# jsourati/nn-active-learning

Measured on AMD Instinct MI355X. Metric: patches/sec Fisher-scored (32^3, 2-class), higher is better.
Workload: dtype f32 (fp32 operands split into 16-bit pieces on the 16-bit MFMA, fp32 accumulate: fp16 pairs - 22-23 bits kept per operand, three products - in the conv under the head (forward + backward), in dec1's forward launch and in the other backward launches; bf16 triples - all 24 bits, exact, six products -

## Files before the change

### nn-active-learning_amd/csrc/alq_internal.h

```cpp
#pragma once
#include <hip/hip_runtime.h>

#include <cstdint>
#include <cstdio>
#include <memory>
#include <string>
#include <vector>

#include "alq.h"

namespace alq {

void set_error(const char *fmt, ...);

#define ALQ_HIP(expr)                                                                     \
    do {                                                                                  \
        hipError_t e_ = (expr);                                                           \
        if (e_ != hipSuccess) {                                                           \
            ::alq::set_error("%s:%d: %s -> %s", __FILE__, __LINE__, #expr,               \
                             hipGetErrorString(e_));                                      \
            return ALQ_EHIP;                                                              \
        }                                                                                 \
    } while (0)

// ... 192 lines not shown
    int mask_split = 0;
    long long mask_delta = 0;
    const unsigned char *mask_bits = nullptr;
    unsigned char *sign_out = nullptr;
    const unsigned *in_bits = nullptr;
    const float *in_vec = nullptr;
    float in_vec_amax = 0.f;
    const unsigned *in_vec16 = nullptr;
    unsigned *out_amax = nullptr;
    int amax_from = 0;
    const unsigned *in_amax = nullptr, *in_amax2 = nullptr;
    float in_bound = 0.f;
    const float *fc_W = nullptr;
    long long fc_F = 0;
    float *fc_part = nullptr;
    unsigned *fc_bits = nullptr;
    unsigned *flip_cnt = nullptr, *flip_list = nullptr;
    int flip_cap = 0;
    float flip_l1 = 0.f;
    bool flip_bias_nonzero = false;
};

extern unsigned long long *g_igemm2_dbg;
constexpr int ALQ_NKNOBS = 10;
extern int g_dbg_knobs[ALQ_NKNOBS];
extern int g_dcp_last_form;
extern int g_no_f16x2;
extern int g_no_fixed;
extern int g_no_xcd_order;
int igemm2_build_plan(const IgemmPlan &p1, Igemm2Plan *p2);
void igemm2_pack_weights(Igemm2Plan *p2, const std::vector<float> &Bmat);
int igemm2_launch(alq_ctx *ctx, const Igemm2Plan &plan, const View &in, const View &out, const float *bias,
                  int relu, int accumulate, int N, int prof_cls, const Igemm2Fuse *fuse);

struct Igemm3Plan {
    bool ok = false;
    bool wres = false;
    int NTW = 1;
    int wgs_per_cu = 1;
    size_t lds_bytes = 0;
    std::vector<unsigned short> h_W;
    void *d_W = nullptr;
    std::vector<unsigned short> h_W16;
    void *d_W16 = nullptr;
    int w16_exp = 0;
};
int igemm3_build_plan(const Igemm2Plan &p2, Igemm3Plan *p3);
// ... 111 lines not shown
                   const float *fc_W, float *fc_part, float *asum_part, unsigned char *fc_bits, float flip_tau);
int c3d_bwd_build(const View &fwd_in, const View &fwd_out, const int k[3], const int lo[3], const int s[3], C3dPlan *plan);
void c3d_bwd_pack(C3dPlan *plan, const std::vector<float> &Bmat_fwd );
void c3d_presplit_vec(const float *v, long long F, int e, std::vector<unsigned short> *out);
int c3d_bwd_launch(alq_ctx *ctx, const C3dPlan &plan, int N, const unsigned char *bits, const void *vec16, int e_in, const unsigned char *maskA,
                   float *dB, float *sumA, float *sumB, int rows_per_wave = 8);

struct T3dPlan {
    bool ok = false;
    int kind = 0;
    int w_exp = 0;
    double flops_per_patch = 0;
    std::vector<unsigned short> h_W;
    void *d_W = nullptr;
};
int t3d_build(const View &in, const View &out, const int k[3], const int lo[3], const int s[3], T3dPlan *fwd, T3dPlan *bwd);
void t3d_fwd_pack(T3dPlan *plan, const float *W );
void t3d_bwd_pack(T3dPlan *plan, const float *W);
void t3d8_fwd_pack(T3dPlan *plan, const float *W );
void t3d8_bwd_pack(T3dPlan *plan, const float *W );
int t3d8_bwd_launch(alq_ctx *ctx, const T3dPlan &plan, const View &dout, const View &din, int N, float in_bound, const unsigned char *mask_bits, float *dsum);
int t3d_fwd_launch(alq_ctx *ctx, const T3dPlan &plan, const View &in, const View &out, const float *bias, int N, float *osum, unsigned *out_amax);
int t3d_bwd_launch(alq_ctx *ctx, const T3dPlan &plan, const View &dout, const View &din, int N, float in_bound, const unsigned char *mask_bits,
                   float *dsum);

struct E3dPlan {
    bool ok = false;
    int w_exp = 0;
    double flops_per_patch = 0;
    std::vector<unsigned short> h_Whi, h_Wlo;
    void *d_Whi = nullptr, *d_Wlo = nullptr;
};
int e3d_build(const View &in, const View &out, const int k[3], const int lo[3], const int s[3], E3dPlan *plan);
void e3d_pack(E3dPlan *plan, const float *W );
int e3d_bwd_launch(alq_ctx *ctx, const E3dPlan &plan, int N, const float *skip, const float *dpool, const unsigned char *am2, const unsigned char *sg2,
                   const unsigned char *am1, const unsigned char *sg1, float *dsum2, float *dsum1, float in_bound,
                   bool rows );

struct D3dPlan {
    bool ok = false;
    int w_exp = 0;
    double flops_per_patch = 0;
    std::vector<unsigned short> h_Whi, h_Wlo;
    void *d_Whi = nullptr, *d_Wlo = nullptr;
    std::vector<unsigned short> h_Bhi, h_Blo;
    void *d_Bhi = nullptr, *d_Blo = nullptr;
};
// ... 222 lines not shown
```

### nn-active-learning_amd/csrc/igemm2.hip

```cpp
#include "alq_internal.h"

#include <algorithm>
#include <cmath>
#include <cstring>

namespace alq {

typedef float f32x4 __attribute__((ext_vector_type(4)));
typedef float f32x2 __attribute__((ext_vector_type(2)));

#ifdef ALQ_STAMPS
#define STAMP(var) asm volatile("s_memtime %0\n\ts_waitcnt lgkmcnt(0)" : "=s"(var)::"memory")
#define PHASE_END(idx)                         \
    do {                                       \
        unsigned long long t_now_;             \
        STAMP(t_now_);                         \
        ph[idx] += t_now_ - t_last;            \
        t_last = t_now_;                       \
    } while (0)
#else
#define PHASE_END(idx) do {} while (0)
#endif

constexpr int I2_CBP = 12;
// ... 461 lines not shown
}

void igemm2_pack_weights(Igemm2Plan *p2, const std::vector<float> &Bmat) {
    const Igemm2Args &a = p2->a;
    const int NTW = p2->NTW, Ci = a.Ci, Co = a.Co;
    p2->h_W.assign((size_t)a.nchunks * a.ntaps * NTW * 128, 0.f);
    for (int ch = 0; ch < a.nchunks; ++ch)
        for (int tp = 0; tp < a.ntaps; ++tp)
            for (int nt = 0; nt < NTW; ++nt)
                for (int lane = 0; lane < 64; ++lane)
                    for (int s = 0; s < 2; ++s) {
                        const int c = ch * 8 + 2 * (lane >> 4) + s;
                        const int co = nt * 16 + (lane & 15);
                        if (co < Co)
                            p2->h_W[((((size_t)ch * a.ntaps + tp) * NTW + nt) * 64 + lane) * 2 + s] =
                                Bmat[((size_t)tp * Ci + c) * Co + co];
                    }
}

unsigned long long *g_igemm2_dbg = nullptr;
int g_no_f16x2 = 0;
int g_no_xcd_order = 0;
int g_no_fixed = 0;
int g_dbg_knobs[ALQ_NKNOBS] = {0, 0, 0, 0, 0, 0, 0, 0, 0, 0};

template <int NTW, bool WRES, int GEO, bool SUMS>
static int launch2_s(alq_ctx *ctx, const Igemm2Plan &plan, const Igemm2Args &a, unsigned grid) {
    auto kfn = igemm2_kernel<NTW, WRES, GEO, SUMS>;
    if (plan.lds_bytes > 64 * 1024)
        ALQ_HIP(hipFuncSetAttribute(reinterpret_cast<const void *>(kfn), hipFuncAttributeMaxDynamicSharedMemorySize,
                                    (int)plan.lds_bytes));
    hipLaunchKernelGGL(kfn, dim3(grid), dim3(256), plan.lds_bytes, ctx->stream, a);
    ALQ_HIP(hipGetLastError());
    return ALQ_OK;
}

template <int NTW, bool WRES, int GEO>
static int launch2_t(alq_ctx *ctx, const Igemm2Plan &plan, const Igemm2Args &a, unsigned grid) {
    return (a.osumA || a.osumB) ? launch2_s<NTW, WRES, GEO, true>(ctx, plan, a, grid)
                                : launch2_s<NTW, WRES, GEO, false>(ctx, plan, a, grid);
}

int igemm2_launch(alq_ctx *ctx, const Igemm2Plan &plan, const View &in, const View &out, const float *bias, int relu,
                  int accumulate, int N, int prof_cls, const Igemm2Fuse *fuse) {
    Igemm2Args a = plan.a;
    ALQ_REQUIRE(in.C == a.Ci && in.D == a.ID && in.H == a.IH && in.W == a.IW, ALQ_EINVAL,
                "igemm2: input view does not match plan");
// ... 53 lines not shown
```

### nn-active-learning_amd/csrc/model.hip

```cpp
#include <algorithm>
#include <cmath>
#include <cstdarg>
#include <cstring>
#include <string>
#include <memory>

#include "alq_internal.h"

namespace alq {

static thread_local char g_err[1024] = "";
void set_error(const char *fmt, ...) {
    va_list ap;
    va_start(ap, fmt);
    vsnprintf(g_err, sizeof(g_err), fmt, ap);
    va_end(ap);
}

int gather_normalize_impl(alq_ctx *, const void *const *, int, int, const int64_t[3], const int64_t[3],
                          const int64_t *, int64_t, const int32_t[3], const double *, int, int, void *);
int score_entropy_impl(alq_ctx *, const float *, int64_t, double *, float *);
int synth_impl(alq_ctx *, uint64_t, int64_t, int64_t, int64_t, float *);
int gather_rows_impl(alq_ctx *, const float *, const int64_t *, int64_t, int64_t, float *);
int debug_view_copy(alq_ctx *, const View &, int, float *);
// ... 91 lines not shown
    int no_flipfix = 0;
    size_t amax_tiles_len = 0;
    int in_dims[4] = {1, 1, 1, 1};
    int nclass = 0;
    int L = 0;
    std::vector<Layer> layers;
    std::vector<void *> allocs;
    float *logits = nullptr, *dlogits = nullptr, *post = nullptr;
    double *S = nullptr, *sizes = nullptr, *Apart = nullptr;
    double *Spart = nullptr;
    int *nslab = nullptr;
    int nslab_max = 1;
    float *wg_partial = nullptr;
    size_t wg_partial_len = 0;
    double *gn_partial = nullptr;
    size_t gn_partial_len = 0;
    double *df_scratch = nullptr;
    double *ls_part = nullptr;
    std::vector<int> ls_nslab;
    int ls_nslab_max = 0;
    int last_lsum = 0;
    float *x_stage = nullptr;
    int64_t epp = 0;
    int knobs[ALQ_NKNOBS] = {0, 0, 0, 0, 0, 0, 0, 0, 0, 0};
    int no_f16x2 = 0;
    int no_xcd_order = 0;
    int requested_batch = 0;
    int no_bound16 = 0;
    int no_fixed = 0;
    int no_presplit = 0;
    int no_signs = 0;
    int no_signs0 = 0;
    int f16_fwd_mask = -1;
    int f16_fwd_derived = 0;
    int no_f16_derived = 0;
    float *d_bound_L = nullptr, *d_bound_B = nullptr;
    int *d_bound_src = nullptr;
    int no_light_kernels = 0;
    int no_c3d = 0;
    int c3_bwd_rows = 8;
    bool last_c3 = false;
    bool last_c3_bwd = false;
    int no_e3d = 0;
    int last_e3b = 0;
    int e3d_rows = 0;
    int last_e3b_form = 0;
    int no_d3d = 0;
    int last_d3f = 0;
    int no_f3d = 0, last_f3f = 0;
    int no_d3b = 0, last_d3b = 0;
    int no_t3d = 0;
    int last_dcp = 0;
    int last_t3f = 0, last_t3b = 0;
    bool last_f16_derived = false;
    int64_t host_pack_elems = 0;
    void *d_wscal = nullptr;
    bool hv_ready = false;
    double *hv_part = nullptr;
    double *hv_p64 = nullptr;

    template <typename T>
    int dalloc(T **p, size_t count) {
        void *q = nullptr;
        const size_t bytes = std::max<size_t>(count * sizeof(T), 256);
        if (hipMalloc(&q, bytes) != hipSuccess) {
            set_error("hipMalloc of %zu bytes failed", bytes);
            return ALQ_ENOMEM;
        }
        allocs.push_back(q);
// ... 35 lines not shown
            s.pool.push_back(pr.first);
            s.pool.push_back(pr.second);
        }
        s.pending.clear();
    }
    return ALQ_OK;
}

static int upload1(alq_model *m, IgemmPlan *p) {
    if (!p->d_W) ALQ_TRY(m->dalloc(&p->d_W, p->h_W.size()));
    ALQ_HIP(hipMemcpyAsync(p->d_W, p->h_W.data(), p->h_W.size() * sizeof(float), hipMemcpyHostToDevice,
                           m->ctx->stream));
    if (p->smallc) {
        if (!p->d_koff) ALQ_TRY(m->dalloc(&p->d_koff, p->h_koff.size()));
        ALQ_HIP(hipMemcpyAsync(p->d_koff, p->h_koff.data(), p->h_koff.size() * sizeof(int),
                               hipMemcpyHostToDevice, m->ctx->stream));
    }
    ALQ_HIP(hipStreamSynchronize(m->ctx->stream));
    std::vector<float>().swap(p->h_W);
    return ALQ_OK;
}

static bool g_use_v2 = true;
static int g_knob_override[ALQ_NKNOBS] = {-1, -1, -1, -1, -1, -1, -1, -1, -1, -1};

static void apply_knobs(const alq_model *m) {
    for (int k = 0; k < ALQ_NKNOBS; ++k) g_dbg_knobs[k] = g_knob_override[k] >= 0 ? g_knob_override[k] : m->knobs[k];
    g_no_f16x2 = m->no_f16x2;
    g_no_xcd_order = m->no_xcd_order;
    g_no_fixed = m->no_fixed;
}

static int gemm_build(const ConvDesc &d, int max_batch, Gemm *g, const G4Geom *g4 = nullptr) {
    ALQ_TRY(igemm_build_plan(d, max_batch, &g->p1));
    if (g4 && !getenv("ALQ_DISABLE_V4")) {
        G4Geom gg = *g4;
        gg.flops_per_patch = g->p1.flops_per_patch;
        ALQ_TRY(igemm4_build_plan(gg, max_batch, &g->p4));
    }
    ALQ_TRY(igemm2_build_plan(g->p1, &g->p2));
    ALQ_TRY(direct_build_plan(g->p1, &g->pd));
    if (!g_use_v2) { g->p2.ok = false; g->pd.ok = false; }
    ALQ_TRY(igemm3_build_plan(g->p2, &g->p3));
    if (d.ID == 1 && d.IH == 1 && d.IW == 1 && d.tz.size() == 1 && d.sm == 1 && d.so == 1 && !getenv("ALQ_NO_FCGEMM"))
        ALQ_TRY(fcgemm_build_plan(d.Ci, d.Co, &g->pfc));
    if (const char *e = getenv("ALQ_DISABLE_V3")) { if (e[0] == '1') g->p3.ok = false; }
    return ALQ_OK;
// ... 911 lines not shown
static int side_join(alq_ctx *c) {
    if (!c->side || !c->side_used) return ALQ_OK;
    c->side_used = false;
    ALQ_HIP(hipEventRecord(c->ev_join, c->side));
    ALQ_HIP(hipStreamWaitEvent(c->stream, c->ev_join, 0));
    return ALQ_OK;
}

static int run_backward_main(alq_model *m, const float *d_x, int N);
static int run_backward(alq_model *m, const float *d_x, int N) {
    const int rc = run_backward_main(m, d_x, N);
    const int rj = side_join(m->ctx);
    return rc != ALQ_OK ? rc : rj;
}

static int run_backward_main(alq_model *m, const float *d_x, int N) {
    alq_ctx *ctx = m->ctx;
    const int nl = (int)m->layers.size();
    ALQ_REQUIRE(m->nclass == 2, ALQ_EUNSUPPORTED, "Fisher scoring is binary (PW_NNAL.py:766), got %d classes", m->nclass);
    ALQ_TRY(k_fill_unit_cotangent(ctx, m->dlogits, N));
    for (Layer &l : m->layers) { l.delta_ready = false; l.dsum_partial = false; l.dout_bits = nullptr; l.dout_vec = nullptr; l.dout_vec16 = nullptr; l.dout_vec16c = nullptr; l.dout_amax = nullptr; }
    m->last_c3_bwd = false;
    m->last_t3b = 0;
    const bool v4_on = !g_dbg_knobs[4] && !g_dbg_knobs[5];
    {
        for (Layer &l : m->layers) l.dout_bound = 0.f;
        m->layers[nl - 1].dout_bound = 1.f;
        for (int i = nl - 1; i >= 1; --i) {
            const Layer &ly = m->layers[i];
            double inb = ly.dout_bound;
            if (ly.spec.type == ALQ_FC)
                inb = (ly.spec.cout == 2 && ly.fc_wv_amax > 0.f && i == nl - 1) ? (double)ly.fc_wv_amax : (i < nl - 1 ? ly.bwd_l1 * ly.dout_bound : 0.0);
            else if (ly.spec.type != ALQ_POOL) inb = ly.bwd_l1 * ly.dout_bound;
            if (!(inb > 0.0) || ly.dout_bound <= 0.f) inb = 0.0;
            auto add = [&](Layer &p) { p.dout_bound = (p.dout_bound < 0.f || inb <= 0.0) ? -1.f : p.dout_bound + (float)(inb * (1.0 + 1e-6)); };
            add(m->layers[i - 1]);
            if (ly.spec.skip_src >= 0) add(m->layers[ly.spec.skip_src]);
        }
    }
    auto pool_first_ok = [&](const Layer &pl, const Layer &src) {
        return pl.spec.type == ALQ_POOL && src.pidx == 0 && src.spec.type != ALQ_FC && pl.spec.k[1] == 2 && pl.spec.k[2] == 2 &&
               (pl.spec.k[0] == 1 || pl.spec.k[0] == 2) && pl.lo[0] == 0 && pl.lo[1] == 0 && pl.lo[2] == 0 &&
               src.out.D == pl.out.D * pl.spec.k[0] && src.out.H == pl.out.H * 2 && src.out.W == pl.out.W * 2 &&
               (pl.out.C == 4 || pl.out.C == 8 || pl.out.C == 16) && ((pl.dout.cs | pl.dout.c0 | pl.out.cs | pl.out.c0) & 3) == 0 &&
               src.spec.relu && !g_dbg_knobs[6];
    };
// ... 154 lines not shown
                }
                if (p4_here && !acc && ly.dout_amax) fz.in_amax = ly.dout_amax;
                if (p4_here && !acc && !fz.in_amax && ly.dout_bound > 0.f && !m->no_bound16) fz.in_bound = ly.dout_bound;
                if (!fuse && !acc && v4_on && ly.bwd.p4.ok && !ly.bwd.p4.multi && ly.bwd.p4.a.PT == 1 && !g_no_f16x2 && !ly.dout_amax &&
                    ly.dout_bound > 0.f && !m->no_bound16 && !g_dbg_knobs[2]) {
                    fz = Igemm2Fuse();
                    fz.in_bound = ly.dout_bound;
                    fuse = &fz;
                }
                if (!ly.bwd.p4.ok && ly.bwd.p3.ok && ly.bwd.p3.d_W16 && !acc && !g_no_f16x2 && ly.dout_bound > 0.f && !m->no_bound16 && !g_dbg_knobs[2] &&
                    !g_dbg_knobs[4] && !g_dbg_knobs[5] && !ly.bwd.pd.ok && !ly.bwd.pfc.ok) {
                    if (!fuse) { fz = Igemm2Fuse(); fuse = &fz; }
                    fz.in_bound = ly.dout_bound;
                }
                const unsigned *mine = ly.dout_amax;
                ly.dout_amax = nullptr;
                const bool t3 = ly.spec.type == ALQ_CONVT && ly.t3b.ok && ly.t3b.d_W && !m->no_t3d && v4_on && !g_no_f16x2 && !acc && fuse && !hand &&
                                fz.in_bound > 0.f && !fz.in_amax && fz.split == 0 && fz.store_from == 0 && fz.osumA && !fz.osumB && fz.mask_from == 0 &&
                                (!fz.mask || fz.mask_bits) && !ly.dout.split && !ly.din.split && prev_param;
                const bool d3 = ly.spec.type == ALQ_CONV && ly.d3f.ok && ly.d3f.d_Bhi && !m->no_d3d && !m->no_d3b && v4_on && !g_no_f16x2 && !acc && fuse && !hand &&
                                fz.in_bound > 0.f && !fz.in_amax && fz.split == 16 && fz.store_from == 0 && !fz.mask && !fz.osumA && fz.osumB &&
                                !ly.dout.split && ly.dout.cs == 16 && ly.dout.c0 == 0 && ly.din.split == 16 && ly.din.cs == 16 && ly.din.c0 == 0 && ly.din.C == 32;
                if (t3) {
                    ALQ_TRY(t3d_bwd_launch(ctx, ly.t3b, ly.dout, ly.din, N, fz.in_bound, fz.mask ? fz.mask_bits : nullptr, fz.osumA));
                    fused = true;
                    m->last_t3b += 1;
                } else if (d3) {
                    ALQ_TRY(d3d_bwd_launch(ctx, ly.d3f, N, ly.dout.p, fz.in_bound, ly.din.p, ly.din.p + ly.din.delta, fz.osumB));
                    fused = true;
                    m->last_d3b = 1;
                } else
                ALQ_TRY(gemm_launch(ctx, ly.bwd, ly.dout, ly.din, nullptr, 0, acc, N, PROF_IGEMM_BWD, fuse, &fused));
                if (hand) {
                    unsigned *dst = mine == m->amax_a ? m->amax_b : m->amax_a;
                    ALQ_TRY(k_rowmax_u32(ctx, m->amax_tiles, ly.bwd.p4.a.tpg * 4, N, dst));
                    prev->dout_amax = dst;
                }
            }
        }
        if (prev_param && fused) prev->delta_ready = true;
    }
    return ALQ_OK;
}

static void clear_fisher_backward_info(alq_model *m) {
    m->last_c3_bwd = false;
    m->last_t3b = 0;
    m->last_e3b = 0;
    m->last_e3b_form = 0;
    m->last_d3b = 0;
}

static int run_backward_general(alq_model *m, int N, const DropSpec *drop, bool layer_sums = false) {
    alq_ctx *ctx = m->ctx;
    const int nl = (int)m->layers.size();
    m->last_lsum = layer_sums ? 1 : 0;
    clear_fisher_backward_info(m);
    for (int i = nl - 1; i >= 0; --i) {
        Layer &ly = m->layers[i];
        const bool isfc = ly.spec.type == ALQ_FC;
        const bool prev_is_src = (i > 0 && m->layers[i - 1].out_is_skip_src && ly.spec.skip_src < 0);
        if (drop && drop->on(i))
            ALQ_TRY(k_dropout(ctx, isfc ? flat_view(ly.dout) : ly.dout, N, drop->first_sample, drop->seed, i, drop->keep_prob));
        if (ly.spec.type == ALQ_POOL) {
            if (i == 0) break;
            bool fused = false;
            ALQ_TRY(k_pool_bwd(ctx, ly.dout, ly.din, ly.argmax, ly.spec.k, ly.lo, N, prev_is_src ? 1 : 0, nullptr, nullptr, &fused, 1));
            continue;
        }
        View dv = isfc ? flat_view(ly.dout) : ly.dout;
// ... 641 lines not shown
    ALQ_REQUIRE(n_layers >= 1 && n_layers <= 64 && max_batch >= 1, ALQ_EINVAL, "alq_model_create: bad sizes");
    ALQ_HIP(hipSetDevice(ctx->device));
    alq_model *m = new alq_model();
    m->ctx = ctx;
    m->max_batch = max_batch;
    {
        const char *e = getenv("ALQ_DISABLE_V2");
        g_use_v2 = !(e && e[0] == '1');
        m->no_f16x2 = getenv("ALQ_NO_F16X2") != nullptr;
        m->no_xcd_order = getenv("ALQ_NO_XCD_ORDER") != nullptr;
        m->no_fixed = getenv("ALQ_NO_FIXED") != nullptr;
        m->no_bound16 = getenv("ALQ_NO_BOUND16") != nullptr;
        m->no_flipfix = getenv("ALQ_NO_FLIPFIX") != nullptr;
        m->no_presplit = getenv("ALQ_NO_PRESPLIT") != nullptr;
        m->no_c3d = getenv("ALQ_NO_C3D") != nullptr;
        m->no_light_kernels = getenv("ALQ_NO_LIGHT_KERNELS") != nullptr;
        { const char *e = getenv("ALQ_C3D_BWD_ROWS"); m->c3_bwd_rows = (e && atoi(e) == 4) ? 4 : ((e && atoi(e) == 8) ? 8 : 7); }
        m->no_signs = getenv("ALQ_NO_SIGNS") != nullptr;
        m->no_signs0 = getenv("ALQ_NO_SIGNS0") != nullptr;
        if (const char *f = getenv("ALQ_F16_FWD_MASK")) m->f16_fwd_mask = atoi(f);
        m->no_t3d = getenv("ALQ_NO_T3D") ? 1 : 0;
        m->no_e3d = getenv("ALQ_NO_E3D") ? 1 : 0;
        { const char *e = getenv("ALQ_E3D_ROWS"); m->e3d_rows = (e && atoi(e) == 1) ? 1 : 0; }
        m->no_d3d = getenv("ALQ_NO_D3D") ? 1 : 0;
        m->no_f3d = getenv("ALQ_NO_F3D") ? 1 : 0;
        m->no_d3b = getenv("ALQ_NO_D3D_BWD") ? 1 : 0;
        {
            const char *e = getenv("ALQ_F16_DERIVED"), *n = getenv("ALQ_NO_F16_DERIVED");
            m->no_f16_derived = ((e && atoi(e) == 0) || (n && atoi(n) == 1)) ? 1 : 0;
        }
        static const char *names[ALQ_NKNOBS] = {"ALQ_DEBUG_REPEAT", "ALQ_DEBUG_FLAGS", "ALQ_NO_BWD_FUSE", "ALQ_NO_FWD_FUSE", "ALQ_NO_V3", "ALQ_NO_V4",
                                                "ALQ_NO_POOL_FIRST", "ALQ_NO_CONV_POOL", "ALQ_DCP_NARROW", "ALQ_E3D_GRID_CAP"};
        for (int k = 0; k < ALQ_NKNOBS; ++k) {
            const char *v = getenv(names[k]);
            if (v) m->knobs[k] = atoi(v);
        }
    }
    for (int i = 0; i < 4; ++i) m->in_dims[i] = in_dims[i];
    m->epp = (int64_t)in_dims[0] * in_dims[1] * in_dims[2] * in_dims[3];
    const int rc = build_model(m, layers, n_layers);
    if (rc != ALQ_OK) {
        alq_model_destroy(m);
        return rc;
    }
    if (const char *t = getenv("ALQ_G4_TUNE")) {
        std::string all(t);
        size_t pos = 0;
        while (pos < all.size()) {
            size_t end = all.find(';', pos);
            if (end == std::string::npos) end = all.size();
            const std::string item = all.substr(pos, end - pos);
            pos = end + 1;
            if (item.size() < 3 || (item[0] != 'f' && item[0] != 'b')) continue;
            const size_t colon = item.find(':');
            if (colon == std::string::npos) continue;
// ... 629 lines not shown
        return ALQ_OK;
    }
    if (what == 0 || what == 1) {
        const Layer &head = m->layers.back();
        ALQ_REQUIRE(!(layer_idx + 2 == (int)m->layers.size() && head.spec.type == ALQ_FC &&
                      (what == 0 ? m->last_head_fused
                                 : (m->last_call_fisher && head.fc_maskbits != nullptr && !g_dbg_knobs[4] && !g_dbg_knobs[5]))),
                    ALQ_EUNSUPPORTED, "layer %d: this tensor is not materialised in a Fisher pass (fc head fused into the layer: "
                    "create the model under ALQ_NO_FC_BITS=1 to keep it)", layer_idx);
        const View &v = what == 0 ? ly.out : ly.dout;
        if (elems_out) *elems_out = (int64_t)N * v.elems();
        return debug_view_copy(m->ctx, v, N, d_out);
    }
    ALQ_REQUIRE(ly.pidx >= 0 && (what == 2 || what == 3), ALQ_EINVAL, "layer has no channel-sum fields");
    const bool isfc = ly.spec.type == ALQ_FC;
    const int64_t e = (int64_t)N * (isfc ? 1 : (what == 2 ? ly.in.vox() : ly.out.vox()));
    if (elems_out) *elems_out = e;
    ALQ_HIP(hipMemcpyAsync(d_out, what == 2 ? ly.asum : ly.dsum, e * sizeof(float), hipMemcpyDeviceToDevice,
                           m->ctx->stream));
    return ALQ_OK;
}

int alq_model_engine_info(alq_model *m, int what) {
    ALQ_REQUIRE(m && ((what >= 0 && what <= 3) || (what >= 5 && what <= 17)), ALQ_EINVAL, "alq_model_engine_info: bad argument");
    if (what == 17) return m->last_e3b_form;
    if (what == 16) return m->last_dcp;
    if (what == 15) return m->last_lsum;
    if (what == 14) return m->host_pack_elems > 0x7fffffffll ? 0x7fffffff : (int)m->host_pack_elems;
    if (what == 13) return m->last_c3_bwd ? m->c3_bwd_rows : 0;
    if (what == 6) return m->last_f16_derived ? 1 : 0;
    if (what == 7) return m->last_t3f;
    if (what == 8) return m->last_t3b;
    if (what == 12) return m->last_f3f;
    if (what == 11) return m->last_d3b;
    if (what == 10) return m->last_d3f;
    if (what == 9) return m->last_e3b;
    ALQ_HIP(hipSetDevice(m->ctx->device));
    if (what == 0) return c3d_subnormals_ok(m->ctx);
    if (what == 1) return m->last_c3 ? 1 : 0;
    if (what == 2) return m->last_c3_bwd ? 1 : 0;
    if (what == 5) {
        if (!m->flip_overflow) return 0;
        unsigned h = 0;
        ALQ_HIP(hipMemcpyAsync(&h, m->flip_overflow, sizeof(unsigned), hipMemcpyDeviceToHost, m->ctx->stream));
        ALQ_HIP(hipStreamSynchronize(m->ctx->stream));
        return h > 0x7fffffffu ? 0x7fffffff : (int)h;
    }
// ... 26 lines not shown
```

### nn-active-learning_amd/csrc/t3d.hip

```cpp
#include "alq_internal.h"
#ifndef T3_CLOBBER
#define T3_CLOBBER : "memory"
#endif

#include <algorithm>
#include <cmath>
#include <cstdlib>
#include <cstring>
#include <vector>

namespace alq {

typedef float f32x4 __attribute__((ext_vector_type(4)));
typedef float f32x2 __attribute__((ext_vector_type(2)));
typedef int i32x4 __attribute__((ext_vector_type(4)));
typedef int i32x2 __attribute__((ext_vector_type(2)));
typedef __bf16 bf16x2 __attribute__((ext_vector_type(2)));
typedef __bf16 bf16x8 __attribute__((ext_vector_type(8)));
typedef _Float16 f16x8 __attribute__((ext_vector_type(8)));
typedef _Float16 f16x2 __attribute__((ext_vector_type(2)));

struct T3FwdArgs {
    const float *in;
    float *out;
// ... 326 lines not shown
#pragma unroll
                for (int pc = 0; pc < 2; ++pc) fo[tz][pc] = fn[tz][0][pc];
            const unsigned crow = ((unsigned)p * 16u + (unsigned)iz) * 16u + (unsigned)iy;
            f32x4 v = f32x4{c.x * a.inv, c.y * a.inv, c.z * a.inv, c.w * a.inv};
            if constexpr (MASK) {
                v.x = (nb & 1u) ? v.x : 0.f; v.y = (nb & 2u) ? v.y : 0.f;
                v.z = (nb & 4u) ? v.z : 0.f; v.w = (nb & 8u) ? v.w : 0.f;
            }
#ifndef T3_NO_OPAQUE
            asm volatile("" : "+v"(v));
#endif
            __builtin_amdgcn_raw_buffer_store_b128(__builtin_bit_cast(i32x4, v), out_rsrc, (int)st_o, (int)(crow * 1024u), 0);
            if constexpr (SUMS) {
                float s = (v.x + v.y) + (v.z + v.w);
                s += __shfl_xor(s, 16, 64);
                s += __shfl_xor(s, 32, 64);
                if (k == 0) s_odd = s;
                else
                    __builtin_amdgcn_raw_buffer_store_b32(__builtin_bit_cast(int, kg == 1 ? s_odd : s), sum_rsrc, (int)sm_o, (int)(crow * 64u), 0);
            }
            __builtin_amdgcn_sched_barrier(0);
            asm volatile("s_nop 3" :: "v"(v) T3_CLOBBER);
        }
    }
}

struct T8FwdArgs {
    const float *in;
    float *out;
    const unsigned short *W;
    const float *bias;
    float *osum;
    int N;
};
constexpr int T8_WBYTES = 27 * 3 * 1024;
constexpr int T8_ROWB = 8 * 64 + 32;
constexpr int T8_SLOT = 3 * T8_ROWB;
constexpr int T8_PLANE = 3 * T8_SLOT;
constexpr int T8_WAVE = 2 * T8_PLANE;

template <bool SUMS>
__global__ __launch_bounds__(512, 2) void t3d8_fwd_kernel(const T8FwdArgs a) {
    extern __shared__ __attribute__((aligned(16))) char t3lds[];
    {
        const i32x4 *src = reinterpret_cast<const i32x4 *>(a.W);
        i32x4 *dst = reinterpret_cast<i32x4 *>(t3lds);
// ... 268 lines not shown
            hipLaunchKernelGGL(kfn, grid8, dim3(512), T8_WBYTES + 8 * T8_WAVE, ctx->stream, a8);
            return ALQ_OK;
        };
        ALQ_TRY(osum ? go(t3d8_fwd_kernel<true>) : go(t3d8_fwd_kernel<false>));
        ALQ_HIP(hipGetLastError());
        return ALQ_OK;
    }
    ALQ_REQUIRE(in.cs == 16 && in.c0 == 0 && in.split == 0 && out.cs == 8 && out.c0 == 0 && out.split == 0 && in.D == 16 && out.D == 32 && bias,
                ALQ_EINVAL, "t3d: view mismatch");
    ALQ_REQUIRE(N < 4096, ALQ_EUNSUPPORTED, "t3d: 32-bit byte offsets hold fewer than 4096 patches per pass");
    if (N <= 0) return ALQ_OK;
    T3FwdArgs a;
    a.in = in.p; a.out = out.p; a.W = reinterpret_cast<const unsigned short *>(plan.d_W); a.bias = bias; a.osum = osum; a.out_amax = out_amax; a.N = N;
    ProfScope ps(ctx, PROF_IGEMM3_FWD, plan.flops_per_patch * N);
    const dim3 grid(t3_grid(ctx, N));
    if (osum && out_amax) hipLaunchKernelGGL((t3d_fwd_kernel<true, true>), grid, dim3(256), 4 * T3F_WAVE, ctx->stream, a);
    else if (osum) hipLaunchKernelGGL((t3d_fwd_kernel<true, false>), grid, dim3(256), 4 * T3F_WAVE, ctx->stream, a);
    else if (out_amax) hipLaunchKernelGGL((t3d_fwd_kernel<false, true>), grid, dim3(256), 4 * T3F_WAVE, ctx->stream, a);
    else hipLaunchKernelGGL((t3d_fwd_kernel<false, false>), grid, dim3(256), 4 * T3F_WAVE, ctx->stream, a);
    ALQ_HIP(hipGetLastError());
    return ALQ_OK;
}

int t3d_bwd_launch(alq_ctx *ctx, const T3dPlan &plan, const View &dout, const View &din, int N, float in_bound, const unsigned char *mask_bits, float *dsum) {
    ALQ_REQUIRE(plan.ok && plan.d_W, ALQ_EINVAL, "t3d: weights not set");
    if (plan.kind == 8) return t3d8_bwd_launch(ctx, plan, dout, din, N, in_bound, mask_bits, dsum);
    ALQ_REQUIRE(dout.cs == 8 && dout.c0 == 0 && dout.split == 0 && din.cs == 16 && din.c0 == 0 && din.split == 0 && din.D == 16 && dout.D == 32 && in_bound > 0.f,
                ALQ_EINVAL, "t3d: view mismatch");
    ALQ_REQUIRE(N < 4096, ALQ_EUNSUPPORTED, "t3d: 32-bit byte offsets hold fewer than 4096 patches per pass");
    if (N <= 0) return ALQ_OK;
    int ex = 0;
    (void)std::frexp(in_bound, &ex);
    const int e_in = 14 - ex;
    T3BwdArgs a;
    a.dout = dout.p; a.din = din.p; a.W = reinterpret_cast<const unsigned short *>(plan.d_W); a.mask_bits = mask_bits; a.dsum = dsum;
    a.scale = std::ldexp(1.f, e_in); a.inv = std::ldexp(1.f, -(e_in + plan.w_exp)); a.N = N;
    ProfScope ps(ctx, PROF_IGEMM_F16, plan.flops_per_patch * N);
    const dim3 grid(t3_grid(ctx, N));
    if (mask_bits && dsum) hipLaunchKernelGGL((t3d_bwd_kernel<true, true>), grid, dim3(256), 4 * T3B_WAVE, ctx->stream, a);
    else if (mask_bits) hipLaunchKernelGGL((t3d_bwd_kernel<true, false>), grid, dim3(256), 4 * T3B_WAVE, ctx->stream, a);
    else if (dsum) hipLaunchKernelGGL((t3d_bwd_kernel<false, true>), grid, dim3(256), 4 * T3B_WAVE, ctx->stream, a);
    else hipLaunchKernelGGL((t3d_bwd_kernel<false, false>), grid, dim3(256), 4 * T3B_WAVE, ctx->stream, a);
    ALQ_HIP(hipGetLastError());
    return ALQ_OK;
}

}
```

Before: 281,500.

## Add plane-sweep backward kernel for t3d transposed conv as default path

Adds a new t3d backward kernel that sweeps z-planes of each patch through a four-slot LDS ring buffer. It uses 512 threads per block, keeps the weights in registers and prefetches the input several planes ahead, so each staged plane feeds three output depth taps instead of being reloaded. This kernel becomes the default path. The previous row-based kernel stays available through ALQ_T3B_ROWS=1, and a new grid-cap knob is added. The cost is a large LDS footprint per block (over 100 KB) and a persistent grid of about one block per CU, which limits occupancy.

```diff
diff --git a/nn-active-learning_amd/csrc/alq_internal.h b/nn-active-learning_amd/csrc/alq_internal.h
--- a/nn-active-learning_amd/csrc/alq_internal.h
+++ b/nn-active-learning_amd/csrc/alq_internal.h
@@ -238,7 +238,7 @@
 };
 
 extern unsigned long long *g_igemm2_dbg;
-constexpr int ALQ_NKNOBS = 10;
+constexpr int ALQ_NKNOBS = 11;
 extern int g_dbg_knobs[ALQ_NKNOBS];
 extern int g_dcp_last_form;
 extern int g_no_f16x2;
@@ -396,7 +396,7 @@
 int t3d8_bwd_launch(alq_ctx *ctx, const T3dPlan &plan, const View &dout, const View &din, int N, float in_bound, const unsigned char *mask_bits, float *dsum);
 int t3d_fwd_launch(alq_ctx *ctx, const T3dPlan &plan, const View &in, const View &out, const float *bias, int N, float *osum, unsigned *out_amax);
 int t3d_bwd_launch(alq_ctx *ctx, const T3dPlan &plan, const View &dout, const View &din, int N, float in_bound, const unsigned char *mask_bits,
-                   float *dsum);
+                   float *dsum, bool rows);
 
 struct E3dPlan {
     bool ok = false;
diff --git a/nn-active-learning_amd/csrc/igemm2.hip b/nn-active-learning_amd/csrc/igemm2.hip
--- a/nn-active-learning_amd/csrc/igemm2.hip
+++ b/nn-active-learning_amd/csrc/igemm2.hip
@@ -507,7 +507,7 @@
 int g_no_f16x2 = 0;
 int g_no_xcd_order = 0;
 int g_no_fixed = 0;
-int g_dbg_knobs[ALQ_NKNOBS] = {0, 0, 0, 0, 0, 0, 0, 0, 0, 0};
+int g_dbg_knobs[ALQ_NKNOBS] = {0, 0, 0, 0, 0, 0, 0, 0, 0, 0, 0};
 
 template <int NTW, bool WRES, int GEO, bool SUMS>
 static int launch2_s(alq_ctx *ctx, const Igemm2Plan &plan, const Igemm2Args &a, unsigned grid) {
diff --git a/nn-active-learning_amd/csrc/model.hip b/nn-active-learning_amd/csrc/model.hip
--- a/nn-active-learning_amd/csrc/model.hip
+++ b/nn-active-learning_amd/csrc/model.hip
@@ -137,7 +137,7 @@
     int last_lsum = 0;
     float *x_stage = nullptr;
     int64_t epp = 0;
-    int knobs[ALQ_NKNOBS] = {0, 0, 0, 0, 0, 0, 0, 0, 0, 0};
+    int knobs[ALQ_NKNOBS] = {0, 0, 0, 0, 0, 0, 0, 0, 0, 0, 0};
     int no_f16x2 = 0;
     int no_xcd_order = 0;
     int requested_batch = 0;
@@ -160,6 +160,8 @@
     int last_e3b = 0;
     int e3d_rows = 0;
     int last_e3b_form = 0;
+    int t3b_rows = 0;
+    int last_t3b_form = 0;
     int no_d3d = 0;
     int last_d3f = 0;
     int no_f3d = 0, last_f3f = 0;
@@ -241,7 +243,7 @@
 }
 
 static bool g_use_v2 = true;
-static int g_knob_override[ALQ_NKNOBS] = {-1, -1, -1, -1, -1, -1, -1, -1, -1, -1};
+static int g_knob_override[ALQ_NKNOBS] = {-1, -1, -1, -1, -1, -1, -1, -1, -1, -1, -1};
 
 static void apply_knobs(const alq_model *m) {
     for (int k = 0; k < ALQ_NKNOBS; ++k) g_dbg_knobs[k] = g_knob_override[k] >= 0 ? g_knob_override[k] : m->knobs[k];
@@ -1199,6 +1201,7 @@
     for (Layer &l : m->layers) { l.delta_ready = false; l.dsum_partial = false; l.dout_bits = nullptr; l.dout_vec = nullptr; l.dout_vec16 = nullptr; l.dout_vec16c = nullptr; l.dout_amax = nullptr; }
     m->last_c3_bwd = false;
     m->last_t3b = 0;
+    m->last_t3b_form = 0;
     const bool v4_on = !g_dbg_knobs[4] && !g_dbg_knobs[5];
     {
         for (Layer &l : m->layers) l.dout_bound = 0.f;
@@ -1399,9 +1402,10 @@
                                 fz.in_bound > 0.f && !fz.in_amax && fz.split == 16 && fz.store_from == 0 && !fz.mask && !fz.osumA && fz.osumB &&
                                 !ly.dout.split && ly.dout.cs == 16 && ly.dout.c0 == 0 && ly.din.split == 16 && ly.din.cs == 16 && ly.din.c0 == 0 && ly.din.C == 32;
                 if (t3) {
-                    ALQ_TRY(t3d_bwd_launch(ctx, ly.t3b, ly.dout, ly.din, N, fz.in_bound, fz.mask ? fz.mask_bits : nullptr, fz.osumA));
+                    ALQ_TRY(t3d_bwd_launch(ctx, ly.t3b, ly.dout, ly.din, N, fz.in_bound, fz.mask ? fz.mask_bits : nullptr, fz.osumA, m->t3b_rows != 0));
                     fused = true;
                     m->last_t3b += 1;
+                    if (ly.t3b.kind == 0) m->last_t3b_form = m->t3b_rows ? 1 : 2;
                 } else if (d3) {
                     ALQ_TRY(d3d_bwd_launch(ctx, ly.d3f, N, ly.dout.p, fz.in_bound, ly.din.p, ly.din.p + ly.din.delta, fz.osumB));
                     fused = true;
@@ -1423,6 +1427,7 @@
 static void clear_fisher_backward_info(alq_model *m) {
     m->last_c3_bwd = false;
     m->last_t3b = 0;
+    m->last_t3b_form = 0;
     m->last_e3b = 0;
     m->last_e3b_form = 0;
     m->last_d3b = 0;
@@ -2110,6 +2115,7 @@
         m->no_t3d = getenv("ALQ_NO_T3D") ? 1 : 0;
         m->no_e3d = getenv("ALQ_NO_E3D") ? 1 : 0;
         { const char *e = getenv("ALQ_E3D_ROWS"); m->e3d_rows = (e && atoi(e) == 1) ? 1 : 0; }
+        { const char *e = getenv("ALQ_T3B_ROWS"); m->t3b_rows = (e && atoi(e) == 1) ? 1 : 0; }
         m->no_d3d = getenv("ALQ_NO_D3D") ? 1 : 0;
         m->no_f3d = getenv("ALQ_NO_F3D") ? 1 : 0;
         m->no_d3b = getenv("ALQ_NO_D3D_BWD") ? 1 : 0;
@@ -2118,7 +2124,7 @@
             m->no_f16_derived = ((e && atoi(e) == 0) || (n && atoi(n) == 1)) ? 1 : 0;
         }
         static const char *names[ALQ_NKNOBS] = {"ALQ_DEBUG_REPEAT", "ALQ_DEBUG_FLAGS", "ALQ_NO_BWD_FUSE", "ALQ_NO_FWD_FUSE", "ALQ_NO_V3", "ALQ_NO_V4",
-                                                "ALQ_NO_POOL_FIRST", "ALQ_NO_CONV_POOL", "ALQ_DCP_NARROW", "ALQ_E3D_GRID_CAP"};
+                                                "ALQ_NO_POOL_FIRST", "ALQ_NO_CONV_POOL", "ALQ_DCP_NARROW", "ALQ_E3D_GRID_CAP", "ALQ_T3B_GRID_CAP"};
         for (int k = 0; k < ALQ_NKNOBS; ++k) {
             const char *v = getenv(names[k]);
             if (v) m->knobs[k] = atoi(v);
@@ -2794,7 +2800,8 @@
 }
 
 int alq_model_engine_info(alq_model *m, int what) {
-    ALQ_REQUIRE(m && ((what >= 0 && what <= 3) || (what >= 5 && what <= 17)), ALQ_EINVAL, "alq_model_engine_info: bad argument");
+    ALQ_REQUIRE(m && ((what >= 0 && what <= 3) || (what >= 5 && what <= 18)), ALQ_EINVAL, "alq_model_engine_info: bad argument");
+    if (what == 18) return m->last_t3b_form;
     if (what == 17) return m->last_e3b_form;
     if (what == 16) return m->last_dcp;
     if (what == 15) return m->last_lsum;
diff --git a/nn-active-learning_amd/csrc/t3d.hip b/nn-active-learning_amd/csrc/t3d.hip
--- a/nn-active-learning_amd/csrc/t3d.hip
+++ b/nn-active-learning_amd/csrc/t3d.hip
@@ -372,6 +372,162 @@
             __builtin_amdgcn_sched_barrier(0);
             asm volatile("s_nop 3" :: "v"(v) T3_CLOBBER);
         }
+    }
+}
+
+constexpr int T3Z_ROW = 2 * T3B_ROWB;
+constexpr int T3Z_IMG = 33 * T3Z_ROW;
+constexpr int T3Z_ZERO = 4 * T3Z_IMG;
+constexpr int T3Z_LDS = T3Z_ZERO + 5 * T3Z_ROW;
+#ifndef T3Z_PF
+#define T3Z_PF 2
+#endif
+static_assert(T3Z_IMG % 16 == 0 && T3Z_LDS <= 160 * 1024, "t3d plane sweep: LDS layout");
+#ifndef T3Z_ABL
+#define T3Z_ABL 0
+#endif
+#ifndef T3Z_NT
+#define T3Z_NT 1
+#endif
+
+template <bool MASK, bool SUMS>
+__global__ __launch_bounds__(512) void t3d_bwdz_kernel(const T3BwdArgs a) {
+    extern __shared__ __attribute__((aligned(16))) char t3lds[];
+    for (int i = threadIdx.x; i < T3Z_LDS / 16; i += 512) reinterpret_cast<i32x4 *>(t3lds)[i] = i32x4{0, 0, 0, 0};
+    __syncthreads();
+    const int lane = threadIdx.x & 63, wave = __builtin_amdgcn_readfirstlane((int)(threadIdx.x >> 6));
+    const int n = lane & 15, kg = lane >> 4;
+    const int w_off = (lane >> 1) * 16 + (lane & 1) * 8 + 4 * wave * T3Z_ROW;
+    const int f_off = (2 * n + kg) * 16;
+    f16x8 wr[9][2];
+#pragma unroll
+    for (int c = 0; c < 9; ++c)
+#pragma unroll
+        for (int pc = 0; pc < 2; ++pc)
+            wr[c][pc] = *reinterpret_cast<const f16x8 *>(a.W + ((size_t)(c * 2 + pc) * 64 + lane) * 8);
+#pragma unroll
+    for (int c = 0; c < 9; ++c)
+#pragma unroll
+        for (int pc = 0; pc < 2; ++pc) asm volatile("" : "+v"(wr[c][pc]));
+    const __amdgpu_buffer_rsrc_t in_rsrc = t3_rsrc(a.dout, (unsigned long long)a.N * 32 * 32 * 32 * 8 * 4);
+    const __amdgpu_buffer_rsrc_t out_rsrc = t3_rsrc(a.din, (unsigned long long)a.N * 16 * 16 * 16 * 16 * 4);
+    const __amdgpu_buffer_rsrc_t sum_rsrc = t3_rsrc(a.dsum, SUMS ? (unsigned long long)a.N * 16 * 16 * 16 * 4 : 0ull);
+    const __amdgpu_buffer_rsrc_t msk_rsrc = t3_rsrc(a.mask_bits, MASK ? (unsigned long long)a.N * 16 * 16 * 16 * 4 : 0ull);
+    const unsigned ld_off = (unsigned)lane * 16u;
+    const unsigned st_off = (T3Z_ABL & 4) ? T3_OOB : (unsigned)n * 64u + (unsigned)kg * 16u;
+    const unsigned mk_off = (unsigned)n * 4u + (unsigned)kg;
+    const unsigned sm_off = ((T3Z_ABL & 4) || kg >= 2) ? T3_OOB : (unsigned)n * 4u + (unsigned)kg * 64u;
+    const float sc = a.scale;
+    const int G = (int)gridDim.x, b0 = (int)blockIdx.x;
+    const int nunits = a.N > b0 ? (a.N - b0 + G - 1) / G : 0;
+    const int T = nunits * 32;
+
+    auto stage = [&](char *dst, const f32x4 &R) __attribute__((always_inline)) {
+        if constexpr (T3Z_ABL & 1) {
+            *reinterpret_cast<i32x2 *>(dst) = i32x2{__builtin_bit_cast(int, R.x), __builtin_bit_cast(int, R.y)};
+            *reinterpret_cast<i32x2 *>(dst + T3B_ROWB) = i32x2{__builtin_bit_cast(int, R.z), __builtin_bit_cast(int, R.w)};
+        } else {
+            const float x0 = R.x * sc, x1 = R.y * sc, x2 = R.z * sc, x3 = R.w * sc;
+            const f16x2 h01 = __builtin_convertvector(f32x2{x0, x1}, f16x2), h23 = __builtin_convertvector(f32x2{x2, x3}, f16x2);
+            const f16x2 l01 = __builtin_convertvector(f32x2{x0 - (float)h01.x, x1 - (float)h01.y}, f16x2);
+            const f16x2 l23 = __builtin_convertvector(f32x2{x2 - (float)h23.x, x3 - (float)h23.y}, f16x2);
+            *reinterpret_cast<i32x2 *>(dst) = i32x2{__builtin_bit_cast(int, h01), __builtin_bit_cast(int, h23)};
+            *reinterpret_cast<i32x2 *>(dst + T3B_ROWB) = i32x2{__builtin_bit_cast(int, l01), __builtin_bit_cast(int, l23)};
+        }
+    };
+    auto fetch = [&](int m, f32x4 *r) __attribute__((always_inline)) {
+        const bool ok = m >= 0 && m < T;
+        const int mc = (ok && !(T3Z_ABL & 2)) ? m : 0;
+        const unsigned row0 = ((((unsigned)b0 + (unsigned)(mc >> 5) * (unsigned)G) * 32u + (unsigned)(mc & 31)) * 32u + (unsigned)(4 * wave)) * 1024u;
+        const unsigned off = ok ? ld_off : T3_OOB;
+#pragma unroll
+        for (int i = 0; i < 4; ++i)
+            r[i] = __builtin_bit_cast(f32x4, __builtin_amdgcn_raw_buffer_load_b128(in_rsrc, (int)off, (int)(row0 + (unsigned)i * 1024u), (T3Z_NT & 1) ? 2 : 0));
+    };
+    f32x4 R[T3Z_PF][4];
+#pragma unroll
+    for (int k = 0; k < T3Z_PF; ++k)
+#pragma unroll
+        for (int i = 0; i < 4; ++i) R[k][i] = f32x4{0.f, 0.f, 0.f, 0.f};
+    static_assert(T3Z_PF == 2 || T3Z_PF == 4, "a pass over the body is T3Z_PF / 2 pairs of sub-steps; the buffer of a sub-step is its position in the pass");
+
+    auto pair = [&](const int t0, f32x4 *Ra, f32x4 *Rb) __attribute__((always_inline)) {
+        const bool live = t0 >= 0;
+        const int o = live ? t0 >> 1 : 0;
+        const int p = b0 + (o >> 4) * G, iz = o & 15;
+        const unsigned st_o = live ? st_off : T3_OOB, sm_o = live ? sm_off : T3_OOB;
+        const unsigned crow = ((unsigned)p * 16u + (unsigned)iz) * 16u + (unsigned)(2 * wave);
+        unsigned nb_o = 0u, nb_e = 0u;
+        f32x4 c_o = f32x4{0.f, 0.f, 0.f, 0.f}, c_e = f32x4{0.f, 0.f, 0.f, 0.f};
+        auto contract = [&](int tz, const char *src) __attribute__((always_inline)) {
+            f16x8 f[5][2];
+#pragma unroll
+            for (int y = 0; y < 5; ++y)
+#pragma unroll
+                for (int pc = 0; pc < 2; ++pc) f[y][pc] = *reinterpret_cast<const f16x8 *>(src + y * T3Z_ROW + pc * T3B_ROWB);
+#pragma unroll
+            for (int ty = 0; ty < 3; ++ty) {
+                const f16x8 *w = wr[tz * 3 + ty];
+                if constexpr (T3Z_ABL & 8) {
+                    asm volatile("" : "+v"(c_o), "+v"(c_e) : "v"(f[ty][0]), "v"(f[ty][1]), "v"(f[ty + 2][0]), "v"(f[ty + 2][1]));
+                } else {
+                    c_o = __builtin_amdgcn_mfma_f32_16x16x32_f16(w[1], f[ty + 2][0], c_o, 0, 0, 0);
+                    c_e = __builtin_amdgcn_mfma_f32_16x16x32_f16(w[1], f[ty][0], c_e, 0, 0, 0);
+                    c_o = __builtin_amdgcn_mfma_f32_16x16x32_f16(w[0], f[ty + 2][1], c_o, 0, 0, 0);
+                    c_e = __builtin_amdgcn_mfma_f32_16x16x32_f16(w[0], f[ty][1], c_e, 0, 0, 0);
+                    c_o = __builtin_amdgcn_mfma_f32_16x16x32_f16(w[0], f[ty + 2][0], c_o, 0, 0, 0);
+                    c_e = __builtin_amdgcn_mfma_f32_16x16x32_f16(w[0], f[ty][0], c_e, 0, 0, 0);
+                }
+            }
+        };
+#pragma unroll
+        for (int b = 0; b < 2; ++b) {
+            __builtin_amdgcn_sched_barrier(0);
+            const int t = t0 + b;
+            asm volatile("s_waitcnt lgkmcnt(0)\n\ts_barrier" ::: "memory");
+            if constexpr (MASK)
+                if (b == 0) {
+                    nb_e = (unsigned)(unsigned char)__builtin_amdgcn_raw_buffer_load_b8(msk_rsrc, (int)(live ? mk_off : T3_OOB), (int)(crow * 64u), 0);
+                    nb_o = (unsigned)(unsigned char)__builtin_amdgcn_raw_buffer_load_b8(msk_rsrc, (int)(live ? mk_off : T3_OOB), (int)(crow * 64u + 64u), 0);
+                }
+            char *dst = t3lds + ((t + 3) & 3) * T3Z_IMG + w_off;
+#pragma unroll
+            for (int i = 0; i < 4; ++i) stage(dst + i * T3Z_ROW, (b ? Rb : Ra)[i]);
+            fetch(t + 3 + T3Z_PF, b ? Rb : Ra);
+            const int rows = f_off + 4 * wave * T3Z_ROW;
+            if (b == 0) contract(0, t3lds + (t0 & 3) * T3Z_IMG + rows);
+            else {
+                contract(1, t3lds + ((t0 + 1) & 3) * T3Z_IMG + rows);
+                contract(2, t3lds + (iz == 15 ? T3Z_ZERO + f_off : ((t0 + 2) & 3) * T3Z_IMG + rows));
+                f32x4 v_o = f32x4{c_o.x * a.inv, c_o.y * a.inv, c_o.z * a.inv, c_o.w * a.inv};
+                f32x4 v_e = f32x4{c_e.x * a.inv, c_e.y * a.inv, c_e.z * a.inv, c_e.w * a.inv};
+                if constexpr (MASK) {
+                    v_o.x = (nb_o & 1u) ? v_o.x : 0.f; v_o.y = (nb_o & 2u) ? v_o.y : 0.f;
+                    v_o.z = (nb_o & 4u) ? v_o.z : 0.f; v_o.w = (nb_o & 8u) ? v_o.w : 0.f;
+                    v_e.x = (nb_e & 1u) ? v_e.x : 0.f; v_e.y = (nb_e & 2u) ? v_e.y : 0.f;
+                    v_e.z = (nb_e & 4u) ? v_e.z : 0.f; v_e.w = (nb_e & 8u) ? v_e.w : 0.f;
+                }
+                asm volatile("" : "+v"(v_o), "+v"(v_e));
+                __builtin_amdgcn_raw_buffer_store_b128(__builtin_bit_cast(i32x4, v_o), out_rsrc, (int)st_o, (int)(crow * 1024u + 1024u), (T3Z_NT & 2) ? 2 : 0);
+                __builtin_amdgcn_raw_buffer_store_b128(__builtin_bit_cast(i32x4, v_e), out_rsrc, (int)st_o, (int)(crow * 1024u), (T3Z_NT & 2) ? 2 : 0);
+                if constexpr (SUMS) {
+                    float s_o = (v_o.x + v_o.y) + (v_o.z + v_o.w);
+                    s_o += __shfl_xor(s_o, 16, 64);
+                    s_o += __shfl_xor(s_o, 32, 64);
+                    float s_e = (v_e.x + v_e.y) + (v_e.z + v_e.w);
+                    s_e += __shfl_xor(s_e, 16, 64);
+                    s_e += __shfl_xor(s_e, 32, 64);
+                    __builtin_amdgcn_raw_buffer_store_b32(__builtin_bit_cast(int, kg == 1 ? s_o : s_e), sum_rsrc, (int)sm_o, (int)(crow * 64u), 0);
+                }
+                __builtin_amdgcn_sched_barrier(0);
+                asm volatile("s_nop 3" :: "v"(v_o), "v"(v_e) T3_CLOBBER);
+            }
+        }
+    };
+    if (T > 0)
+    for (int t0 = T3Z_PF == 2 ? -6 : -8; t0 < T; t0 += T3Z_PF) {
+        pair(t0, R[0], R[1]);
+        if constexpr (T3Z_PF == 4) pair(t0 + 2, R[2], R[3]);
     }
 }
 
@@ -686,7 +842,7 @@
     return ALQ_OK;
 }
 
-int t3d_bwd_launch(alq_ctx *ctx, const T3dPlan &plan, const View &dout, const View &din, int N, float in_bound, const unsigned char *mask_bits, float *dsum) {
+int t3d_bwd_launch(alq_ctx *ctx, const T3dPlan &plan, const View &dout, const View &din, int N, float in_bound, const unsigned char *mask_bits, float *dsum, bool rows) {
     ALQ_REQUIRE(plan.ok && plan.d_W, ALQ_EINVAL, "t3d: weights not set");
     if (plan.kind == 8) return t3d8_bwd_launch(ctx, plan, dout, din, N, in_bound, mask_bits, dsum);
     ALQ_REQUIRE(dout.cs == 8 && dout.c0 == 0 && dout.split == 0 && din.cs == 16 && din.c0 == 0 && din.split == 0 && din.D == 16 && dout.D == 32 && in_bound > 0.f,
@@ -700,6 +856,22 @@
     a.dout = dout.p; a.din = din.p; a.W = reinterpret_cast<const unsigned short *>(plan.d_W); a.mask_bits = mask_bits; a.dsum = dsum;
     a.scale = std::ldexp(1.f, e_in); a.inv = std::ldexp(1.f, -(e_in + plan.w_exp)); a.N = N;
     ProfScope ps(ctx, PROF_IGEMM_F16, plan.flops_per_patch * N);
+    if (!rows) {
+        long long g = std::min<long long>(ctx->num_cus, N);
+        g = std::max<long long>(8, (g + 7) / 8 * 8);
+        if (g_dbg_knobs[10] > 0) g = std::min<long long>(g, g_dbg_knobs[10]);
+        auto go = [&](auto kfn) -> int {
+            ALQ_HIP(hipFuncSetAttribute(reinterpret_cast<const void *>(kfn), hipFuncAttributeMaxDynamicSharedMemorySize, T3Z_LDS));
+            hipLaunchKernelGGL(kfn, dim3((unsigned)g), dim3(512), (size_t)T3Z_LDS, ctx->stream, a);
+            return ALQ_OK;
+        };
+        if (mask_bits && dsum) ALQ_TRY(go(t3d_bwdz_kernel<true, true>));
+        else if (mask_bits) ALQ_TRY(go(t3d_bwdz_kernel<true, false>));
+        else if (dsum) ALQ_TRY(go(t3d_bwdz_kernel<false, true>));
+        else ALQ_TRY(go(t3d_bwdz_kernel<false, false>));
+        ALQ_HIP(hipGetLastError());
+        return ALQ_OK;
+    }
     const dim3 grid(t3_grid(ctx, N));
     if (mask_bits && dsum) hipLaunchKernelGGL((t3d_bwd_kernel<true, true>), grid, dim3(256), 4 * T3B_WAVE, ctx->stream, a);
     else if (mask_bits) hipLaunchKernelGGL((t3d_bwd_kernel<true, false>), grid, dim3(256), 4 * T3B_WAVE, ctx->stream, a);
```

Result: no change. 283,900, median of 6 (+0.9%).
